# matssteinweg/Multi-Purpose-MPC

Measured on AMD Instinct MI355X. Metric: MPC QP solves/sec (batch, horizon N=30), higher is better.
Workload: dtype f64

## Files before the change

### multi-purpose-mpc_amd/csrc/mpmpc_reduced.hpp

```cpp
#pragma once
#include "mpmpc_core.hpp"

namespace mpmpc {

inline bool reduced_native(const mpmpc_config& c, const mpmpc_settings& st) {
  return st.native != 0 && reducible(c, st) && st.early_polish == 1 && st.max_iter > 1 && st.ipm_start_mu > 0.0 &&
         st.early_scaling >= 0 && st.scaling > 0;
}

template <class L, bool CR = true>
struct ReducedSolver : Solver<L, false, true, false, CR> {
  using S = Solver<L, false, true, false, CR>;
  using R = typename L::real;
  using Mk = typename L::mask;
  using I = typename L::ival;
  using S::N; using S::n_inst; using S::off_; using S::vx; using S::vu; using S::first; using S::down_chain; using S::is_mid;
  using S::is_end; using S::vxc; using S::sU; using S::val3; using S::bU; using S::live; using S::a; using S::b; using S::mI;
  using S::leq; using S::status; using S::iters; using S::ipm_iters; using S::polished; using S::pri_res; using S::dua_res;
  static constexpr bool kSplit = S::kSplit;
  static constexpr int LAY_RED = S::LAY_RED, LAY_REDSPLIT = S::LAY_REDSPLIT;
  static constexpr int LAY_IP = kSplit ? LAY_REDSPLIT : LAY_RED;
  static constexpr int EI = kSplit ? 2 : 3;
  using Box3 = typename S::template BoxT<LAY_RED>;
  using BoxI = typename S::template BoxT<LAY_IP>;
// ... 24 lines not shown
    n_inst = B;
    live = inst < B;
    vx = live & within_(k, 0, N);
    vu = live & within_(k, 0, N - 1);
    first = (k == 0);
    {
      const int C = L::split;
      off_ = lane_offset(L::group, C, N);
      I kl = k + off_;
      down_chain = (kl >= C);
      is_mid = (kl == C - 1);
      is_end = (kl == 2 * C - 1);
      I kc = seli(down_chain & (kl < 2 * C), kl * (-1) + (3 * C - 1), kl) - off_;
      vxc = live & within_(kc, 0, N);
      if constexpr (kSplit) {
        sU = (kl >= 32);
        Mk vU = live & within_(kl, 32 + off_, N + 31 + off_);
        val3[0] = selb(sU, vU, vx); val3[1] = selb(sU, vU, vx); val3[2] = vx & !sU;
      }
    }
    val[0] = vx; val[1] = vx; val[2] = vu;
  }
  MPMPC_HD void setup_problem(const R* fields, const SolverParams& st) {
    auto fld = [&](int f, double dflt) { return sel(vx, fields[f], R(dflt)); };
    const R zero(0.0), onec(1.0);
    const R lo_v = max_(fld(F_LO + 3, -INFTY), R(-INFTY)), hi_v = min_(fld(F_HI + 3, INFTY), R(INFTY));
    const R p_v = fld(F_P + 3, 1.0), q_v = fld(F_Q + 3, 0.0);
    R v = -q_v / p_v;
    v = sel((hi_v < R(INF_BOUND)) & (v > hi_v), hi_v, v);
    v = sel((lo_v > R(-INF_BOUND)) & (v < lo_v), lo_v, v);
    v = sel(vu, v, zero);
    L::cold_put(C_V, v);
    L::cold_put(C_LAMV, sel(vu, -fma_(p_v, v, q_v), zero));
    L::cold_put(C_A20, fld(F_A20, 0.0));
    L::cold_put(C_BV, fld(F_B20, 0.0) * v);
    L::cold_put(C_BEQ2, fld(F_BEQ + 2, 0.0));
    const R lo_e = max_(fld(F_LO + 0, -INFTY), R(-INFTY)), hi_e = min_(fld(F_HI + 0, INFTY), R(INFTY));
    const R lo_k = max_(fld(F_LO + 4, -INFTY), R(-INFTY)), hi_k = min_(fld(F_HI + 4, INFTY), R(INFTY));
    {
      R gap = max_(max_(sel(vx, lo_e - hi_e, zero), sel(vu, lo_k - hi_k, zero)), sel(vu, lo_v - hi_v, zero));
      gap = L::gmax(gap);
      empty = live & (gap > zero);
      solvable = live & !empty;
      L::cold_put(C_GAP, gap);
    }
    const R ds = fld(F_DS, 0.0), one = sel(vu, onec, zero);
    a[0] = one; a[1] = ds; a[2] = fld(F_A10, 0.0); a[3] = one;
    b[0] = ds;
    mI[0] = mI[1] = R(-1.0);
    P3[0] = fld(F_P + 0, 1.0); P3[1] = fld(F_P + 1, 1.0); P3[2] = fld(F_P + 4, 1.0);
    Q3[0] = fld(F_Q + 0, 0.0); Q3[1] = fld(F_Q + 1, 0.0); Q3[2] = fld(F_Q + 4, 0.0);
    R D3[3] = {onec, onec, onec}, G3[3] = {onec, onec, onec}, Eb[3] = {onec, onec, onec}, E2[2] = {onec, onec}, c3(1.0);
    const int passes = st.early_scaling > 0 && st.early_scaling < st.scaling ? st.early_scaling : st.scaling;
    const R inv_n_total(1.0 / double(3 * N + 2));
    for (int it = 0; it < passes; ++it) {
      R cn[3], rn[2], r_own[2];
      cn[0] = max_(max_(max_(abs_(P3[0]), abs_(mI[0])), max_(abs_(a[0]), abs_(a[2]))), abs_(G3[0]));
      cn[1] = max_(max_(max_(abs_(P3[1]), abs_(mI[1])), max_(abs_(a[1]), abs_(a[3]))), abs_(G3[1]));
      cn[2] = max_(max_(abs_(P3[2]), abs_(b[0])), abs_(G3[2]));
      r_own[0] = max_(abs_(a[0]), abs_(a[1]));
      r_own[1] = max_(max_(abs_(a[2]), abs_(a[3])), abs_(b[0]));
      R Dt[3], Et[2], Etb[3], Etd[2];
      MPMPC_UNROLL
      for (int i = 0; i < 2; ++i) {
        rn[i] = max_(abs_(mI[i]), L::up(r_own[i]));
        Et[i] = rsqrt_(S::limit(rn[i]));
        Etd[i] = L::down(Et[i]);
      }
      MPMPC_UNROLL
      for (int e = 0; e < 3; ++e) {
        Dt[e] = rsqrt_(S::limit(cn[e]));
        Etb[e] = rsqrt_(S::limit(abs_(G3[e])));
        P3[e] = (Dt[e] * P3[e]) * Dt[e];
        G3[e] = (Etb[e] * G3[e]) * Dt[e];
        Q3[e] = Dt[e] * Q3[e];
        D3[e] = D3[e] * Dt[e];
        Eb[e] = Eb[e] * Etb[e];
      }
      MPMPC_UNROLL
      for (int i = 0; i < 2; ++i) { mI[i] = (Et[i] * mI[i]) * Dt[i]; E2[i] = E2[i] * Et[i]; }
      a[0] = (Etd[0] * a[0]) * Dt[0]; a[1] = (Etd[0] * a[1]) * Dt[1];
      a[2] = (Etd[1] * a[2]) * Dt[0]; a[3] = (Etd[1] * a[3]) * Dt[1];
      b[0] = (Etd[1] * b[0]) * Dt[2];
      R s(0.0), mq(0.0);
      MPMPC_UNROLL
      for (int e = 0; e < 3; ++e) {
        s = s + sel(val[e], abs_(P3[e]), zero);
        mq = max_(mq, sel(val[e], abs_(Q3[e]), zero));
      }
      R ct = L::gsum(s) * inv_n_total;
      const R nq = S::limit(L::gmax(mq));
      ct = rcp_(S::limit(max_(ct, nq)));
      MPMPC_UNROLL
      for (int e = 0; e < 3; ++e) { P3[e] = P3[e] * ct; Q3[e] = Q3[e] * ct; }
      c3 = c3 * ct;
    }
    leq[0] = E2[0] * fld(F_BEQ + 0, 0.0);
    leq[1] = E2[1] * fld(F_BEQ + 1, 0.0);
    MPMPC_UNROLL
    for (int e = 0; e < 3; ++e) { L::cold_put(C_D + e, D3[e]); L::cold_put(C_G + e, G3[e]); }
    L::cold_put(C_E, E2[0]); L::cold_put(C_E + 1, E2[1]);
    L::cold_put(C_C, c3);
    {
      const R i0 = rcp_(D3[0]), i2 = rcp_(D3[2]);
      L::cold_put(K_LO0, lo_e * i0); L::cold_put(K_HI0, hi_e * i0); L::cold_put(K_LO2, lo_k * i2); L::cold_put(K_HI2, hi_k * i2);
    }
    MPMPC_UNROLL
    for (int e = 0; e < 3; ++e) {
      x3[e] = zero;
      L::cold_put(C_PI + e, zero);
    }
    L::fence();
  }

  MPMPC_HD void to_ip(const R v[3], R* o, double fill = 0.0) const {
    if constexpr (kSplit) {
      o[0] = sel(sU, L::from_lower(v[2]), v[0]);
      o[1] = sel(sU, R(fill), v[1]);
    } else {
      o[0] = v[0]; o[1] = v[1]; o[2] = v[2];
    }
  }
  MPMPC_HD void from_ip(const R* v, R o[3]) const {
    if constexpr (kSplit) {
      o[0] = v[0]; o[1] = v[1]; o[2] = L::from_upper(v[0]);
    } else {
      o[0] = v[0]; o[1] = v[1]; o[2] = v[2];
    }
  }
  MPMPC_HD void mask_to_ip(const Mk m[3], Mk* o) const {
    if constexpr (kSplit) {
      R v[3], w[2];
      MPMPC_UNROLL
      for (int e = 0; e < 3; ++e) v[e] = sel(m[e], R(1.0), R(0.0));
      to_ip(v, w);
      o[0] = w[0] > R(0.5); o[1] = w[1] > R(0.5);
    } else {
      o[0] = m[0]; o[1] = m[1]; o[2] = m[2];
    }
  }
  MPMPC_HD void mask_from_ip(const Mk* m, Mk o[3]) const {
    if constexpr (kSplit) {
      R w[2] = {sel(m[0], R(1.0), R(0.0)), sel(m[1], R(1.0), R(0.0))}, v[3];
      from_ip(w, v);
      MPMPC_UNROLL
      for (int e = 0; e < 3; ++e) o[e] = v[e] > R(0.5);
    } else {
      o[0] = m[0]; o[1] = m[1]; o[2] = m[2];
    }
  }

  template <bool SOFT = false>
  MPMPC_HD Mk ipm3(const Box3& bx, typename S::template IpmT<LAY_RED>& s, const SolverParams& st, double tol, const Mk& run, int band_slot = -1) {
    const R reg(st.ipm_reg), ireg(st.inv_ipm_reg), one(1.0), zero(0.0);
    constexpr int JB[2] = {0, 2};
    Mk active = run, conv = L::mfalse();
    R cnt(0.0);
    MPMPC_UNROLL
    for (int b = 0; b < 2; ++b) cnt = cnt + L::gcount(bx.Lm[JB[b]]) + L::gcount(bx.Um[JB[b]]);
    const R inb = rcp_(max_(cnt, one));
    I stall(0);
    R mu_min(1e300);
    auto lo_of = [&](int b) { return L::cold_get(b == 0 ? K_LO0 : K_LO2); };
    auto hi_of = [&](int b) { return L::cold_get(b == 0 ? K_HI0 : K_HI2); };
    auto iom_of = [&](int j) { const R gj = L::cold_get(C_G + j); return rcp_(gj * gj); };
    auto w_of = [&](int j) { return SOFT ? (s.zl[j] - s.zu[j]) * iom_of(j) : zero; };
    auto rl_of = [&](int b) { const int j = JB[b]; return SOFT ? s.x[j] + w_of(j) - lo_of(b) - s.sl[j] : s.x[j] - lo_of(b) - s.sl[j]; };
    auto ru_of = [&](int b) { const int j = JB[b]; return SOFT ? hi_of(b) - s.x[j] - w_of(j) - s.su[j] : hi_of(b) - s.x[j] - s.su[j]; };
    auto rpin_of = [&](int b) { const int j = JB[b]; return sel(bx.pin[j], s.x[j] - lo_of(b), zero); };
    auto rpin_raw = [&](int b) { const int j = JB[b]; return s.x[j] - lo_of(b); };
    for (int it = 0; it <= st.ipm_max_iter; ++it) {
      R mu;
      {
        L::fence();
        R At[3], rp[2], rd[3];
        this->template AeqT_mul_t<LAY_RED>(s.nu, At);
        this->template Aeq_mul_t<LAY_RED>(s.x, rp);
        R res(0.0), msum(0.0);
        MPMPC_UNROLL
        for (int i = 0; i < 2; ++i) {
          rp[i] = rp[i] - L::cold_get(K_LEQ + i);
          if constexpr (SOFT) rp[i] = fma_(R(-P1_EQ_SOFT), s.nu[i], rp[i]);
          res = max_(res, sel(vx, abs_(rp[i]), zero));
        }
        MPMPC_UNROLL
        for (int j = 0; j < 3; ++j) {
          if constexpr (SOFT) rd[j] = At[j] - s.zl[j] + s.zu[j] + s.pi[j];
          else rd[j] = fma_(L::cold_get(K_PP + j), s.x[j], L::cold_get(K_QQ + j)) + At[j] - s.zl[j] + s.zu[j] + s.pi[j];
        }
        res = max_(res, sel(val[1], abs_(rd[1]), zero));
        MPMPC_UNROLL
        for (int b = 0; b < 2; ++b) {
          const int j = JB[b];
          res = max_(res, sel(val[j], max_(max_(abs_(rd[j]), abs_(rpin_of(b))), max_(sel(bx.Lm[j], abs_(rl_of(b)), zero), sel(bx.Um[j], abs_(ru_of(b)), zero))), zero));
          msum = msum + s.sl[j] * s.zl[j] + s.su[j] * s.zu[j];
        }
        MPMPC_UNROLL
        for (int j = 0; j < 3; ++j) L::cold_put(K_RD + j, rd[j]);
        L::cold_put(K_RP, rp[0]); L::cold_put(K_RP + 1, rp[1]);
        res = L::gmax(res);
        mu = L::gsum(msum) * inb;
        Mk ok = (res < R(tol > 1e-11 ? tol : 1e-11)) & (mu < R(tol));
        if constexpr (SOFT) {
          S::p1_converged = selb(active, ok, S::p1_converged);
          R ny(0.0), na(0.0), sup(0.0);
          MPMPC_UNROLL
          for (int i = 0; i < 2; ++i) { ny = max_(ny, sel(vx, abs_(s.nu[i]), zero)); sup = sup + sel(vx, L::cold_get(K_LEQ + i) * s.nu[i], zero); }
          na = max_(na, sel(val[0], abs_(rd[0]), zero));
          na = max_(na, sel(val[1], abs_(rd[1]), zero));
          na = max_(na, sel(val[2], abs_(rd[2]), zero));
          MPMPC_UNROLL
          for (int b = 0; b < 2; ++b) {
            const int j = JB[b];
            const R lam = s.zu[j] - s.zl[j] + s.pi[j];
            ny = max_(ny, sel(val[j], abs_(lam), zero));
            sup = sup + sel(val[j] & (lam > zero) & (bx.Um[j] | bx.pin[j]), sel(bx.pin[j], lo_of(b), hi_of(b)) * lam, zero) +
                  sel(val[j] & (lam < zero) & (bx.Lm[j] | bx.pin[j]), lo_of(b) * lam, zero);
          }
          ny = L::gmax(ny); na = L::gmax(na); sup = L::gsum(sup);
          const R thr = R(st.phase1_eps) * ny;
          Mk ray = (ny > R(st.phase1_eps)) & (na < thr) & (sup < -thr);
          if (band_slot >= 0) {
            R wv(0.0);
            MPMPC_UNROLL
            for (int b = 0; b < 2; ++b) {
              const int j = JB[b];
              wv = max_(wv, sel(val[j], abs_(w_of(j)) * L::cold_get(C_D + j), zero));
            }
            ray = ray & (L::gmax(wv) > L::cold_get(band_slot));
          }
          ok = ok | ray;
        }
        conv = conv | (active & ok);
        active = active & !ok;
        if (it == st.ipm_max_iter || !L::wany(active)) break;
        if constexpr (!SOFT) {
          active = active & !(mu > R(st.ipm_diverged) * mu_min) & !((mu < R(tol * 1e-3)) & (res > R(1e-5)));
          mu_min = min_(mu_min, mu);
          if (!L::wany(active)) break;
        }
      }
      ipm_iters = seli(active, ipm_iters + I(1), ipm_iters);
      R isl[2], isu[2], rcl[2], rcu[2];
      [[maybe_unused]] R kap[2];
      {
        L::fence();
        R h[3];
        h[1] = SOFT ? rcp_(reg) : rcp_(L::cold_get(K_PP + 1) + reg);
        MPMPC_UNROLL
        for (int b = 0; b < 2; ++b) {
          const int j = JB[b];
          const R il = rcp_(s.sl[j]), iu = rcp_(s.su[j]);
          if constexpr (SOFT) {
            const R th = sel(bx.Lm[j], s.zl[j] * il, zero) + sel(bx.Um[j], s.zu[j] * iu, zero);
            const R kp = rcp_(fma_(th, iom_of(j), one));
            h[j] = rcp_(fma_(kp, th, reg) + sel(bx.pin[j], ireg, zero));
          } else {
            h[j] = rcp_(L::cold_get(K_PP + j) + reg + sel(bx.Lm[j], s.zl[j] * il, zero) + sel(bx.Um[j], s.zu[j] * iu, zero) +
                        sel(bx.pin[j], ireg, zero));
          }
        }
        this->template factor_t<LAY_RED>(h, SOFT ? reg + R(P1_EQ_SOFT) : reg);
        L::fence();
        MPMPC_UNROLL
        for (int b = 0; b < 2; ++b) {
          const int j = JB[b];
          isl[b] = sel(bx.Lm[j], rcp_(s.sl[j]), zero); isu[b] = sel(bx.Um[j], rcp_(s.su[j]), zero);
          rcl[b] = s.sl[j] * s.zl[j]; rcu[b] = s.su[j] * s.zu[j];
          if constexpr (SOFT) kap[b] = rcp_(fma_(s.zl[j] * isl[b] + s.zu[j] * isu[b], iom_of(j), one));
        }
      }
      R alpha_aff(1.0);
      for (int pass = 0; pass < 2; ++pass) {
        R dx[3], dnu[2];
        [[maybe_unused]] R cul[2];
        {
          L::fence();
          R rhs[3], nreq[2];
          rhs[1] = -L::cold_get(K_RD + 1);
          MPMPC_UNROLL
          for (int b = 0; b < 2; ++b) {
            const int j = JB[b];
            if constexpr (SOFT) {
              cul[b] = fma_(s.zu[j], ru_of(b), rcu[b]) * isu[b] - fma_(s.zl[j], rl_of(b), rcl[b]) * isl[b];
              rhs[j] = fma_(kap[b], cul[b], -L::cold_get(K_RD + j)) - sel(bx.pin[j], rpin_raw(b) * ireg, zero);
            } else {
              rhs[j] = -L::cold_get(K_RD + j) - fma_(s.zl[j], rl_of(b), rcl[b]) * isl[b] + fma_(s.zu[j], ru_of(b), rcu[b]) * isu[b] -
                       sel(bx.pin[j], rpin_raw(b) * ireg, zero);
            }
          }
          nreq[0] = -L::cold_get(K_RP); nreq[1] = -L::cold_get(K_RP + 1);
          this->template kkt_solve_t<LAY_RED>(rhs, nreq, dx, dnu);
          if (SOFT && pass == 1) {
            R Ad[2], Atd[3], r1[3], r2[2];
            this->template Aeq_mul_t<LAY_RED>(dx, Ad);
            this->template AeqT_mul_t<LAY_RED>(dnu, Atd);
            r1[1] = rhs[1] - Atd[1];
            MPMPC_UNROLL
            for (int b = 0; b < 2; ++b) {
              const int j = JB[b];
              r1[j] = rhs[j] - fma_(kap[b] * (s.zl[j] * isl[b] + s.zu[j] * isu[b]) + sel(bx.pin[j], ireg, zero), dx[j], Atd[j]);
            }
            r2[0] = fma_(R(P1_EQ_SOFT), dnu[0], nreq[0] - Ad[0]); r2[1] = fma_(R(P1_EQ_SOFT), dnu[1], nreq[1] - Ad[1]);
            L::fence();
            MPMPC_UNROLL
            for (int j = 0; j < 3; ++j) L::cold_put(K_RD + j, dx[j]);
// ... 403 lines not shown
```

### multi-purpose-mpc_amd/csrc/mpmpc_reduced_tail.hpp

```cpp
#pragma once
#include "mpmpc_reduced.hpp"

namespace mpmpc {

inline bool reduced_native_tail(const mpmpc_config& c, const mpmpc_settings& st) {
  return reduced_native(c, st) && st.phase1 != 0;
}

template <class L, bool CR = true>
struct ReducedTailSolver : ReducedSolver<L, CR> {
  using RS = ReducedSolver<L, CR>;
  using S = typename RS::S;
  using R = typename L::real;
  using Mk = typename L::mask;
  using I = typename L::ival;
  using S::N; using S::vx; using S::vu; using S::first; using S::live; using S::a; using S::b; using S::mI; using S::leq;
  using S::status; using S::iters; using S::ipm_iters; using S::polished; using S::pri_res; using S::dua_res;
  using S::sU; using S::val3; using S::bU;
  using RS::val; using RS::P3; using RS::Q3; using RS::x3; using RS::solvable; using RS::empty;
  using RS::C_D; using RS::C_E; using RS::C_C; using RS::K_LO0; using RS::K_HI0; using RS::K_LO2; using RS::K_HI2; using RS::C_V;
  using RS::C_LAMV; using RS::C_A20; using RS::C_BV; using RS::C_BEQ2; using RS::C_G; using RS::C_PI; using RS::C_XS; using RS::C_LAM;
  using RS::C_NUS; using RS::C_GAP;
  using Box3 = typename RS::Box3;
  using BoxI = typename RS::BoxI;
  using IpmI = typename RS::IpmI;
  static constexpr int EI = RS::EI;
  enum { T_RAW0 = 37, T_RAW1 = 38, T_RAW2 = 39, T_RAW3 = RS::C_PI, T_NAX = RS::C_PI + 1, T_RD0 = RS::C_PI + 2, T_MARK = RS::C_GAP,
         T_BAND = RS::C_NUS };
  static_assert(RS::K_RP + 2 <= 37, "the packed interior point's residual slots must end below T_RAW0");
  MPMPC_HD static constexpr int t_raw(int i) { return i == 0 ? T_RAW0 : (i == 1 ? T_RAW1 : (i == 2 ? T_RAW2 : T_RAW3)); }


  MPMPC_HD void setup_full(const R* fields, int B, const I& inst, const I& k, int N_, const SolverParams& st) {
    RS::context(B, inst, k, N_);
    auto fld = [&](int f, double dflt) { return sel(vx, fields[f], R(dflt)); };
    const R zero(0.0), onec(1.0);
    const R lo_v = max_(fld(F_LO + 3, -INFTY), R(-INFTY)), hi_v = min_(fld(F_HI + 3, INFTY), R(INFTY));
    const R p_v = fld(F_P + 3, 1.0), q_v = fld(F_Q + 3, 0.0);
    R v = -q_v / p_v;
    v = sel((hi_v < R(INF_BOUND)) & (v > hi_v), hi_v, v);
    v = sel((lo_v > R(-INF_BOUND)) & (v < lo_v), lo_v, v);
    v = sel(vu, v, zero);
    L::cold_put(C_V, v);
    L::cold_put(C_LAMV, sel(vu, -fma_(p_v, v, q_v), zero));
    L::cold_put(C_A20, fld(F_A20, 0.0));
    L::cold_put(C_BV, fld(F_B20, 0.0) * v);
    L::cold_put(C_BEQ2, fld(F_BEQ + 2, 0.0));
    const R lo_e = max_(fld(F_LO + 0, -INFTY), R(-INFTY)), hi_e = min_(fld(F_HI + 0, INFTY), R(INFTY));
    const R lo_k = max_(fld(F_LO + 4, -INFTY), R(-INFTY)), hi_k = min_(fld(F_HI + 4, INFTY), R(INFTY));
    {
      R gap = max_(max_(sel(vx, lo_e - hi_e, zero), sel(vu, lo_k - hi_k, zero)), sel(vu, lo_v - hi_v, zero));
      gap = L::gmax(gap);
      empty = live & (gap > zero);
      solvable = live & !empty;
      pri_res = gap;
      L::cold_put(T_MARK, zero);
    }
    {
      auto fin = [&](const R& bnd) { return sel(abs_(bnd) < R(INF_BOUND), abs_(bnd), zero); };
      R m = sel(vx, max_(fin(lo_e), fin(hi_e)), zero);
      m = max_(m, sel(vu, max_(max_(fin(lo_v), fin(hi_v)), max_(abs_(v), max_(fin(lo_k), fin(hi_k)))), zero));
      L::cold_put(T_NAX, L::gmax(m));
      R mb = sel(vx, max_(fin(lo_e), fin(hi_e)), zero);
      mb = max_(mb, sel(vu, max_(max_(fin(lo_v), fin(hi_v)), max_(fin(lo_k), fin(hi_k))), zero));
      L::cold_put(T_BAND, st.phase1_accept ? R(st.phase1_band) * fma_(R(st.eps_rel), L::gmax(mb), R(st.eps_abs)) : zero);
    }
    const R ds = fld(F_DS, 0.0), one = sel(vu, onec, zero);
    S::valid[0] = S::valid[1] = S::valid[2] = vx;
    S::valid[3] = S::valid[4] = vu;
    a[0] = one; a[1] = ds; a[2] = fld(F_A10, 0.0); a[3] = one; a[4] = fld(F_A20, 0.0); a[5] = one;
    b[0] = ds; b[1] = fld(F_B20, 0.0);
    MPMPC_UNROLL
    for (int i = 0; i < 3; ++i) { mI[i] = R(-1.0); S::Eeq[i] = onec; }
    MPMPC_UNROLL
    for (int j = 0; j < 5; ++j) {
      S::q[j] = fld(F_Q + j, 0.0);
      S::p[j] = fld(F_P + j, 1.0);
      S::g[j] = onec; S::D[j] = onec; S::Eb[j] = onec;
    }
    S::c = onec;
    const int passes = st.early_scaling > 0 && st.early_scaling < st.scaling ? st.early_scaling : st.scaling;
    S::ruiz(passes, live);
    constexpr int J5[3] = {0, 1, 4};
    MPMPC_UNROLL
    for (int e = 0; e < 3; ++e) {
      P3[e] = S::p[J5[e]]; Q3[e] = S::q[J5[e]];
      L::cold_put(C_D + e, S::D[J5[e]]);
      L::cold_put(C_G + e, S::g[J5[e]]);
      x3[e] = zero;
    }
    L::cold_put(T_RAW0, lo_e); L::cold_put(T_RAW1, hi_e); L::cold_put(T_RAW2, lo_k); L::cold_put(T_RAW3, hi_k);
    leq[0] = S::Eeq[0] * fld(F_BEQ + 0, 0.0);
    leq[1] = S::Eeq[1] * fld(F_BEQ + 1, 0.0);
    L::cold_put(C_E, S::Eeq[0]); L::cold_put(C_E + 1, S::Eeq[1]);
    L::cold_put(C_C, S::c);
    L::cold_put(K_LO0, (S::Eb[0] * lo_e) / S::g[0]); L::cold_put(K_HI0, (S::Eb[0] * hi_e) / S::g[0]);
    L::cold_put(K_LO2, (S::Eb[4] * lo_k) / S::g[4]); L::cold_put(K_HI2, (S::Eb[4] * hi_k) / S::g[4]);
    L::cold_put(T_RD0, L::gmax(sel(vu, abs_(fma_(S::p[3], v / S::D[3], S::q[3])), zero)));
    L::fence();
  }

  MPMPC_HD R violation(const R xs[3]) const {
    const R zero(0.0);
    R Ax[2], pv(0.0);
    this->template Aeq_mul_t<RS::LAY_RED>(xs, Ax);
    MPMPC_UNROLL
    for (int i = 0; i < 2; ++i) pv = max_(pv, sel(vx, abs_((Ax[i] - leq[i]) / L::cold_get(C_E + i)), zero));
    MPMPC_UNROLL
    for (int b2 = 0; b2 < 2; ++b2) {
      const int e = b2 == 0 ? 0 : 2;
      const R xu = L::cold_get(C_D + e) * xs[e];
      pv = max_(pv, sel(val[e], max_(max_(L::cold_get(t_raw(2 * b2)) - xu, xu - L::cold_get(t_raw(2 * b2 + 1))), zero), zero));
    }
    return L::gmax(pv);
  }

  MPMPC_HD void run(const R* fields, int B, const I& inst, const I& k, int N_, const SolverParams& st, const I& base_ipm) {
    MPMPC_TICK_BEGIN(0);
    setup_full(fields, B, inst, k, N_, st);
    MPMPC_TICK_END(0);
    const R zero(0.0), one(1.0);
    status = seli(empty, I(MPMPC_PRIMAL_INFEASIBLE), I(MPMPC_UNSOLVED));
    ipm_iters = base_ipm;
    polished = I(0);
    pri_res = sel(empty, pri_res, zero);
    dua_res = zero;
    this->act_bits = I(0);
    const Mk todo = solvable;
    if (L::wany(todo)) {
      Box3 b3;
      RS::make_box3(b3);
      R xs[3], lam[3], nus[2];
      {
        const R theta(st.phase1_theta);
        R sl[3], su[3], zl[3], zu[3];
        MPMPC_UNROLL
        for (int e = 0; e < 3; ++e) {
          const R ge = L::cold_get(C_G + e), ig = one / ge;
          sl[e] = sel(b3.Lm[e], max_(-(b3.lo[e] * ge), theta) * ig, one);
          su[e] = sel(b3.Um[e], max_(b3.hi[e] * ge, theta) * ig, one);
          zl[e] = sel(b3.Lm[e], theta * ge, zero);
          zu[e] = sel(b3.Um[e], theta * ge, zero);
        }
        BoxI bi;
        IpmI si;
        Mk vm[EI];
        if constexpr (RS::kSplit) {
          bU[0] = sel(sU, L::from_lower(b[0]), zero);
          bU[1] = zero;
          vm[0] = val3[0]; vm[1] = val3[2];
        } else {
          vm[0] = val[0]; vm[1] = val[1]; vm[2] = val[2];
        }
        RS::to_ip(b3.lo, bi.lo); RS::to_ip(b3.hi, bi.hi);
        RS::mask_to_ip(b3.Lm, bi.Lm); RS::mask_to_ip(b3.Um, bi.Um); RS::mask_to_ip(b3.pin, bi.pin);
        const R z3[3] = {zero, zero, zero};
        RS::to_ip(z3, si.x); RS::to_ip(sl, si.sl, 1.0); RS::to_ip(su, si.su, 1.0); RS::to_ip(zl, si.zl); RS::to_ip(zu, si.zu); RS::to_ip(z3, si.pi);
        si.nu[0] = si.nu[1] = zero;
        MPMPC_UNROLL
        for (int e = 0; e < EI; ++e) si.tL[e] = si.tU[e] = L::mfalse();
        S::p1_converged = L::mfalse();
        MPMPC_TICK_BEGIN(9);
        const double tol1 = st.ipm_tol * 1e-2 < 1e-11 ? st.ipm_tol * 1e-2 : 1e-11;
        if constexpr (RS::kSplit) {
          R om3[3], omI[EI];
          MPMPC_UNROLL
          for (int e = 0; e < 3; ++e) { const R ge = L::cold_get(C_G + e); om3[e] = ge * ge; }
          RS::to_ip(om3, omI, 1.0);
          R d3[3], dI[EI];
          MPMPC_UNROLL
          for (int e = 0; e < 3; ++e) d3[e] = L::cold_get(C_D + e) / om3[e];
          RS::to_ip(d3, dI, 1.0);
          S::p1_band = L::cold_get(T_BAND);
          this->template ipm<RS::LAY_IP, true>(bi, si, omI, dI, vm, st, tol1, todo);
        } else {
          MPMPC_UNROLL
          for (int e = 0; e < 3; ++e) { L::cold_put(RS::K_PP + e, P3[e]); L::cold_put(RS::K_QQ + e, Q3[e]); }
          L::cold_put(RS::K_LEQ, leq[0]); L::cold_put(RS::K_LEQ + 1, leq[1]);
          L::fence();
          RS::template ipm3<true>(bi, si, st, tol1, todo, st.phase1_accept ? (int)T_BAND : -1);
          L::fence();
          MPMPC_UNROLL
// ... 122 lines not shown
```

### multi-purpose-mpc_amd/csrc/mpmpc_solver_polish.hpp

```cpp
#ifndef MPMPC_SOLVER_BODY
#error "include mpmpc_core.hpp"
#endif
  template <int LAY>
  MPMPC_HD Mk active_set(const BoxT<LAY>& bx, const R* pp, const R* qq, const Mk* vm, Mk* aL, Mk* aU, R* xs, R* nus, R* lam,
                         const SolverParams& st, const Mk& run, double add_fraction) {
    constexpr int E = EN<LAY>, NQ = NR<LAY>;
    const R delta(st.as_delta), idelta(st.inv_as_delta), zero(0.0), one(1.0), tol(1e-9);
    Mk todo = run, okm = L::mfalse();
    for (int rnd = 0; rnd < st.as_rounds; ++rnd) {
      if (!L::wany(todo)) break;
      R bound[E];
      Mk act[E];
      MPMPC_UNROLL
      for (int j = 0; j < E; ++j) act[j] = aL[j] | aU[j] | bx.pin[j];
      {
        R h[E], Hd[E];
        MPMPC_UNROLL
        for (int j = 0; j < E; ++j) {
          Hd[j] = pp[j] + delta + sel(act[j], idelta, zero);
          h[j] = one / Hd[j];
        }
        dense_blocks<LAY>(Hd, h);
        MPMPC_TICK_COUNT(17);
        MPMPC_TICK_BEGIN(13);
        factor_t<LAY>(h, delta);
        MPMPC_TICK_END(13);
      }
      L::fence();
      MPMPC_UNROLL
      for (int j = 0; j < E; ++j) bound[j] = sel(aU[j], bx.hi[j], bx.lo[j]);
      R xn[E], nn[NQ], ln[E];
      MPMPC_UNROLL
      for (int j = 0; j < E; ++j) xn[j] = ln[j] = zero;
      MPMPC_UNROLL
      for (int i = 0; i < NQ; ++i) nn[i] = zero;
      [[maybe_unused]] Mk refine = todo;
      for (int rf = 0; rf <= st.as_refine; ++rf) {
        R At[E], Ax[NQ], rhs[E], r2[NQ], r3[E], dx[E], dnu[NQ];
        AeqT_mul_t<LAY>(nn, At);
        Aeq_mul_t<LAY>(xn, Ax);
        R rs(0.0);
        [[maybe_unused]] R Pod[E];
        if constexpr (FQ) {
          MPMPC_UNROLL
          for (int j = 0; j < E; ++j) Pod[j] = zero;
          Poff_add<LAY>(xn, Pod);
        }
        [[maybe_unused]] R rk_dot(0.0);
        if constexpr (LAY == LAY_RED4) rk_dot = rank_one_dot(xn);
        MPMPC_UNROLL
        for (int j = 0; j < E; ++j) {
          R r1 = -qq[j] - pp[j] * xn[j] - At[j] - ln[j];
          if constexpr (FQ) r1 = r1 - Pod[j];
          if constexpr (LAY == LAY_RED4) { if (j == 0 || j == 3) r1 = fma_(-rk_c[j == 0 ? 0 : 1], rk_dot, r1); }
          r3[j] = sel(act[j], bound[j] - xn[j], zero);
          rhs[j] = fma_(r3[j], idelta, r1);
          rs = max_(rs, sel(vm[j], max_(abs_(r1), abs_(r3[j])), zero));
        }
        MPMPC_UNROLL
        for (int i = 0; i < NQ; ++i) { r2[i] = leq[i] - Ax[i]; rs = max_(rs, sel(vx, abs_(r2[i]), zero)); }
        [[maybe_unused]] Mk need = todo;
        if constexpr (L::per_wave == 1) {
          if (rf >= 1 && !L::wany(todo & (L::gmax(rs) > R(1e-15)))) break;
        } else {
          if (rf >= 1) need = refine & (L::gmax(rs) > R(1e-15));
          if (!L::wany(need)) break;
        }
        MPMPC_TICK_COUNT(18);
        MPMPC_TICK_BEGIN(14);
        kkt_solve_t<LAY>(rhs, r2, dx, dnu);
        MPMPC_TICK_END(14);
        R big(0.0);
        MPMPC_UNROLL
        for (int j = 0; j < E; ++j) {
          ln[j] = updw(need, ln[j] + sel(act[j], (dx[j] - r3[j]) * idelta, zero), ln[j]);
          xn[j] = updw(need, xn[j] + dx[j], xn[j]);
          big = max_(big, sel(vm[j], abs_(dx[j]) - R(1e-14) * abs_(xn[j]), zero));
        }
        MPMPC_UNROLL
        for (int i = 0; i < NQ; ++i) nn[i] = updw(need, nn[i] + dnu[i], nn[i]);
        if constexpr (L::per_wave == 1) {
          if (rf >= 1 && !L::wany(todo & (L::gmax(big) > R(1e-15)))) break;
        } else {
          refine = rf < 1 ? need : need & (L::gmax(big) > R(1e-15));
          if (!L::wany(refine)) break;
        }
        if (L::per_wave == 1 && rf >= 1 && rf < st.as_refine) {
          const R far(1e-6);
          Mk clear = L::mfalse();
          MPMPC_UNROLL
          for (int j = 0; j < E; ++j)
            clear = clear | (bx.Lm[j] & !aL[j] & (xn[j] < bx.lo[j] - far)) | (bx.Um[j] & !aU[j] & (xn[j] > bx.hi[j] + far)) |
                    (aL[j] & (ln[j] > far)) | (aU[j] & (ln[j] < -far));
          if (!L::wany(todo & !L::gany(clear))) break;
        }
      }
      Mk anybad = L::mfalse();
      Mk vL[E], vU[E], bL[E], bU_[E];
      R worst(0.0);
      MPMPC_UNROLL
      for (int j = 0; j < E; ++j) {
        vL[j] = bx.Lm[j] & !aL[j] & (xn[j] < bx.lo[j] - tol);
        vU[j] = bx.Um[j] & !aU[j] & (xn[j] > bx.hi[j] + tol);
        bL[j] = aL[j] & (ln[j] > tol);
        bU_[j] = aU[j] & (ln[j] < -tol);
        anybad = anybad | vL[j] | vU[j] | bL[j] | bU_[j];
        worst = max_(worst, max_(sel(vL[j], bx.lo[j] - xn[j], zero), sel(vU[j], xn[j] - bx.hi[j], zero)));
      }
      anybad = L::gany(anybad);
      {
        const R thr = R(add_fraction) * L::gmax(worst);
        MPMPC_UNROLL
        for (int j = 0; j < E; ++j) {
          vL[j] = vL[j] & !(bx.lo[j] - xn[j] < thr);
          vU[j] = vU[j] & !(xn[j] - bx.hi[j] < thr);
        }
      }
      MPMPC_UNROLL
      for (int j = 0; j < E; ++j) {
        xs[j] = updw(todo, xn[j], xs[j]);
        lam[j] = updw(todo, ln[j], lam[j]);
        Mk nL = (aL[j] & !bL[j]) | vL[j];
        Mk nU = ((aU[j] & !bU_[j]) | vU[j]) & !nL;
        aL[j] = selb(todo & anybad, nL, aL[j]);
        aU[j] = selb(todo & anybad, nU, aU[j]);
      }
      MPMPC_UNROLL
      for (int i = 0; i < NQ; ++i) nus[i] = updw(todo, nn[i], nus[i]);
      okm = okm | (todo & !anybad);
      todo = todo & anybad;
    }
    return okm;
  }

  MPMPC_HD void reduced_complete(const Box& bx, R xs[5], R nus[3], R lam[5]) const {
    const R zero(0.0);
    R xv = -q[3] / p[3];
    xv = sel(bx.Um[3] & (xv > bx.hi[3]), bx.hi[3], xv);
    xv = sel((bx.Lm[3] | bx.pin[3]) & (xv < bx.lo[3]), bx.lo[3], xv);
    xv = sel(bx.pin[3], bx.lo[3], xv);
    xs[3] = sel(valid[3], xv, zero);
    lam[3] = sel(valid[3], -fma_(p[3], xs[3], q[3]), zero);
    nus[2] = zero;
    lam[2] = zero;
    const R imI = R(1.0) / mI[2], t0 = leq[2] * imI, drive = fma_(b[1], xs[3], a[4] * xs[0]);
    R t = t0;
    for (int it = 0; it < N; ++it) {
      const R inflow = L::up(fma_(a[5], t, drive));
      t = sel(first, t0, (leq[2] - inflow) * imI);
    }
    xs[2] = sel(vx, t, zero);
  }

  MPMPC_HD Mk certificate(const R xs[5], const R nus[3], const R lam[5], double tol, R& prim, R& stat) const {
    R Ax[3], At[5];
    Aeq_mul(xs, Ax);
    AeqT_mul(nus, At);
    R pv(0.0), sv(0.0), cv(0.0);
    R cinv = R(1.0) / c;
    R Pod[5] = {R(0.0), R(0.0), R(0.0), R(0.0), R(0.0)};
    if constexpr (FQ) Poff_add<0>(xs, Pod);
    MPMPC_UNROLL
    for (int i = 0; i < 3; ++i) pv = max_(pv, sel(vx, abs_((Ax[i] - leq[i]) / Eeq[i]), R(0.0)));
    MPMPC_UNROLL
    for (int j = 0; j < 5; ++j) {
      R xu = D[j] * xs[j];
      const R lo0 = lo_raw(j), hi0 = hi_raw(j);
      R viol = max_(max_(lo0 - xu, xu - hi0), R(0.0));
      pv = max_(pv, sel(valid[j], viol, R(0.0)));
      R rd = fma_(p[j], xs[j], q[j]) + At[j] + lam[j];
      if constexpr (FQ) rd = rd + Pod[j];
      sv = max_(sv, sel(valid[j], abs_(rd / D[j]) * cinv, R(0.0)));
      R yu = (lam[j] / D[j]) * cinv;
      Mk fu = hi0 < R(INF_BOUND), fl = lo0 > R(-INF_BOUND);
      R cu = sel(fu, max_(yu, R(0.0)) * abs_(hi0 - xu), sel(yu > R(0.0), R(1e300), R(0.0)));
      R cl = sel(fl, max_(-yu, R(0.0)) * abs_(xu - lo0), sel(yu < R(0.0), R(1e300), R(0.0)));
      cv = max_(cv, sel(valid[j], max_(cu, cl), R(0.0)));
    }
    Mk bad = L::mfalse();
    MPMPC_UNROLL
    for (int j = 0; j < 5; ++j) bad = bad | (valid[j] & !((abs_(xs[j]) < R(1e300)) & (abs_(lam[j]) < R(1e300))));
    MPMPC_UNROLL
    for (int i = 0; i < 3; ++i) bad = bad | (vx & !(abs_(nus[i]) < R(1e300)));
    bad = L::gany(bad);
    prim = L::gmax(pv);
    stat = L::gmax(sv);
    cv = L::gmax(cv);
    return (prim <= R(tol)) & (stat <= R(tol)) & (cv <= R(tol)) & !bad;
  }

  MPMPC_HD void stash() const {
    MPMPC_UNROLL
    for (int j = 0; j < 5; ++j) {
      L::cold_put(j, D[j]); L::cold_put(5 + j, Eb[j]); L::cold_put(10 + j, lb[j]); L::cold_put(15 + j, ub[j]);
      L::cold_put(20 + j, x[j]); L::cold_put(25 + j, yb[j]); L::cold_put(37 + j, g[j]);
    }
    MPMPC_UNROLL
    for (int i = 0; i < 3; ++i) { L::cold_put(30 + i, Eeq[i]); L::cold_put(33 + i, yeq[i]); }
    L::cold_put(36, c);
    L::fence();
  }
  MPMPC_HD void unstash() {
    L::fence();
    MPMPC_UNROLL
    for (int j = 0; j < 5; ++j) {
      D[j] = L::cold_get(j); Eb[j] = L::cold_get(5 + j); lb[j] = L::cold_get(10 + j); ub[j] = L::cold_get(15 + j);
      x[j] = L::cold_get(20 + j); yb[j] = L::cold_get(25 + j); g[j] = L::cold_get(37 + j);
    }
    MPMPC_UNROLL
    for (int i = 0; i < 3; ++i) { Eeq[i] = L::cold_get(30 + i); yeq[i] = L::cold_get(33 + i); }
    c = L::cold_get(36);
  }

  MPMPC_HD static I pack_active(const Mk aL[5], const Mk aU[5]) {
    I v(1 << 30);
    MPMPC_UNROLL
    for (int j = 0; j < 5; ++j) v = v + seli(aL[j], I(1 << j), I(0)) + seli(aU[j], I(32 << j), I(0));
    return v;
  }
  static constexpr int LAY_AS = RED ? LAY_RED : LAY_FULL;
  static constexpr int LAY_IP = RED ? (kSplit ? LAY_REDSPLIT : LAY_RED) : (kSplit ? LAY_SPLIT : LAY_FULL);

  template <int LAY>
  MPMPC_HD void problem_in_layout(const Box& bx, BoxT<LAY>& bi, R* pp, R* qq, Mk* vm) {
    constexpr int E = EN<LAY>;
    const R one(1.0), zero(0.0);
    if constexpr (SPL<LAY>) {
      MPMPC_UNROLL
      for (int i = 0; i < 2; ++i) bU[i] = sel(sU, L::from_lower(b[i]), zero);
      if constexpr (FQ) {
        podS[0] = sel(sU, L::from_lower(rod), pod[0]); podS[1] = sel(sU, zero, pod[1]); podS[2] = sel(sU, zero, pod[2]);
      }
    }
    to_lay<LAY>(bx.lo, bi.lo); to_lay<LAY>(bx.hi, bi.hi); to_lay<LAY>(p, pp); to_lay<LAY>(q, qq);
    mask_to_lay<LAY>(bx.Lm, bi.Lm); mask_to_lay<LAY>(bx.Um, bi.Um); mask_to_lay<LAY>(bx.pin, bi.pin);
    valid_lay<LAY>(vm);
    if constexpr (LAY == LAY_SPLIT) pp[2] = sel(sU, one, pp[2]);
    if constexpr (LAY == LAY_REDSPLIT) pp[1] = sel(sU, one, pp[1]);
    (void)E;
  }
  template <int LAY>
  MPMPC_HD void iterate_to_layout(const Ipm& s, IpmT<LAY>& si) const {
    const R one(1.0);
    to_lay<LAY>(s.x, si.x); to_lay<LAY>(s.sl, si.sl); to_lay<LAY>(s.su, si.su);
    to_lay<LAY>(s.zl, si.zl); to_lay<LAY>(s.zu, si.zu); to_lay<LAY>(s.pi, si.pi);
    if constexpr (LAY == LAY_SPLIT) { si.sl[2] = sel(sU, one, si.sl[2]); si.su[2] = sel(sU, one, si.su[2]); }
    if constexpr (LAY == LAY_REDSPLIT) { si.sl[1] = sel(sU, one, si.sl[1]); si.su[1] = sel(sU, one, si.su[1]); }
    MPMPC_UNROLL
    for (int i = 0; i < NR<LAY>; ++i) si.nu[i] = s.nu[i];
  }

  MPMPC_HD Mk active_set_full(const Box& bx, Mk aL5[5], Mk aU5[5], R xs[5], R nus[3], R lam[5], const SolverParams& st, double add_fraction,
                              const Mk& run) {
    constexpr int LAY = LAY_AS;
    constexpr int E = EN<LAY>, NQ = NR<LAY>;
    BoxT<LAY> ba;
    R pp[E], qq[E], xa[E], la[E], na[NQ];
    Mk vm[E], aL[E], aU[E];
    problem_in_layout<LAY>(bx, ba, pp, qq, vm);
    mask_to_lay<LAY>(aL5, aL); mask_to_lay<LAY>(aU5, aU);
    to_lay<LAY>(xs, xa); to_lay<LAY>(lam, la);
    MPMPC_UNROLL
    for (int i = 0; i < NQ; ++i) na[i] = nus[i];
    Mk okm = active_set<LAY>(ba, pp, qq, vm, aL, aU, xa, na, la, st, run, add_fraction);
    from_lay<LAY>(xa, xs); from_lay<LAY>(la, lam);
    MPMPC_UNROLL
    for (int i = 0; i < NQ; ++i) nus[i] = na[i];
    mask_from_lay<LAY>(aL, aL5); mask_from_lay<LAY>(aU, aU5);
    if constexpr (RED) {
      reduced_complete(bx, xs, nus, lam);
      aL5[2] = aU5[2] = L::mfalse();
      aL5[3] = bx.Lm[3] & (lam[3] < R(0.0)) & valid[3];
      aU5[3] = bx.Um[3] & (lam[3] > R(0.0)) & valid[3] & !aL5[3];
    }
    return okm;
  }

  MPMPC_HD void warm_polish(const SolverParams& st, const I& guess, const Mk& run) {
    Box bx;
    make_box(bx);
    Mk aL[5], aU[5];
    MPMPC_UNROLL
    for (int j = 0; j < 5; ++j) {
      aL[j] = bx.Lm[j] & bit_(guess, j);
// ... 139 lines not shown
```

Baseline: 70.44 million.

## Let each packed instance run its own active-set rounds independently within a wave

```diff
diff --git a/multi-purpose-mpc_amd/csrc/mpmpc_reduced.hpp b/multi-purpose-mpc_amd/csrc/mpmpc_reduced.hpp
--- a/multi-purpose-mpc_amd/csrc/mpmpc_reduced.hpp
+++ b/multi-purpose-mpc_amd/csrc/mpmpc_reduced.hpp
@@ -200,6 +200,7 @@
 
   template <bool SOFT = false>
   MPMPC_HD Mk ipm3(const Box3& bx, typename S::template IpmT<LAY_RED>& s, const SolverParams& st, double tol, const Mk& run, int band_slot = -1) {
+    static_assert(!(SOFT && kLean), "phase 1 needs the full cold storage");
     const R reg(st.ipm_reg), ireg(st.inv_ipm_reg), one(1.0), zero(0.0);
     constexpr int JB[2] = {0, 2};
     Mk active = run, conv = L::mfalse();
diff --git a/multi-purpose-mpc_amd/csrc/mpmpc_reduced_tail.hpp b/multi-purpose-mpc_amd/csrc/mpmpc_reduced_tail.hpp
--- a/multi-purpose-mpc_amd/csrc/mpmpc_reduced_tail.hpp
+++ b/multi-purpose-mpc_amd/csrc/mpmpc_reduced_tail.hpp
@@ -28,6 +28,7 @@
   enum { T_RAW0 = 37, T_RAW1 = 38, T_RAW2 = 39, T_RAW3 = RS::C_PI, T_NAX = RS::C_PI + 1, T_RD0 = RS::C_PI + 2, T_MARK = RS::C_GAP,
          T_BAND = RS::C_NUS };
   static_assert(RS::K_RP + 2 <= 37, "the packed interior point's residual slots must end below T_RAW0");
+  static_assert(!RS::kLean && T_RAW2 < L::cold_slots, "the tail solver needs the full cold storage: its own slots are the last three");
   MPMPC_HD static constexpr int t_raw(int i) { return i == 0 ? T_RAW0 : (i == 1 ? T_RAW1 : (i == 2 ? T_RAW2 : T_RAW3)); }
 
 
diff --git a/multi-purpose-mpc_amd/csrc/mpmpc_solver_polish.hpp b/multi-purpose-mpc_amd/csrc/mpmpc_solver_polish.hpp
--- a/multi-purpose-mpc_amd/csrc/mpmpc_solver_polish.hpp
+++ b/multi-purpose-mpc_amd/csrc/mpmpc_solver_polish.hpp
@@ -4,6 +4,7 @@
   template <int LAY>
   MPMPC_HD Mk active_set(const BoxT<LAY>& bx, const R* pp, const R* qq, const Mk* vm, Mk* aL, Mk* aU, R* xs, R* nus, R* lam,
                          const SolverParams& st, const Mk& run, double add_fraction) {
+    if constexpr (kOwnRounds) { return active_set_own<LAY>(bx, pp, qq, vm, aL, aU, xs, nus, lam, st, run, add_fraction); }
     constexpr int E = EN<LAY>, NQ = NR<LAY>;
     const R delta(st.as_delta), idelta(st.inv_as_delta), zero(0.0), one(1.0), tol(1e-9);
     Mk todo = run, okm = L::mfalse();
@@ -130,6 +131,143 @@
       okm = okm | (todo & !anybad);
       todo = todo & anybad;
     }
+    return okm;
+  }
+
+  static constexpr bool kOwnRounds = L::per_wave > 1 && !kS2;
+  template <int LAY>
+  MPMPC_HD Mk active_set_own(const BoxT<LAY>& bx, const R* pp, const R* qq, const Mk* vm, Mk* aL, Mk* aU, R* xs, R* nus, R* lam,
+                             const SolverParams& st, const Mk& run, double add_fraction) {
+    constexpr int E = EN<LAY>, NQ = NR<LAY>;
+    const R delta(st.as_delta), idelta(st.inv_as_delta), zero(0.0), one(1.0), tol(1e-9);
+    Mk todo = st.as_rounds > 0 ? run : L::mfalse(), okm = L::mfalse();
+    const Mk ran = todo;
+    Mk fresh = todo;
+    I rnd(0), rf(0);
+    R xn[E], nn[NQ], ln[E];
+    MPMPC_UNROLL
+    for (int j = 0; j < E; ++j) xn[j] = ln[j] = zero;
+    MPMPC_UNROLL
+    for (int i = 0; i < NQ; ++i) nn[i] = zero;
+    while (L::wany(todo)) {
+      Mk act[E];
+      MPMPC_UNROLL
+      for (int j = 0; j < E; ++j) act[j] = aL[j] | aU[j] | bx.pin[j];
+      if (L::wany(fresh)) {
+        {
+          R h[E], Hd[E];
+          MPMPC_UNROLL
+          for (int j = 0; j < E; ++j) {
+            Hd[j] = pp[j] + delta + sel(act[j], idelta, zero);
+            h[j] = one / Hd[j];
+          }
+          dense_blocks<LAY>(Hd, h);
+          MPMPC_TICK_COUNT(17);
+          MPMPC_TICK_BEGIN(13);
+          factor_t<LAY>(h, delta);
+          MPMPC_TICK_END(13);
+        }
+        L::fence();
+        MPMPC_UNROLL
+        for (int j = 0; j < E; ++j) { xn[j] = sel(fresh, zero, xn[j]); ln[j] = sel(fresh, zero, ln[j]); }
+        MPMPC_UNROLL
+        for (int i = 0; i < NQ; ++i) nn[i] = sel(fresh, zero, nn[i]);
+        rf = seli(fresh, I(0), rf);
+        fresh = L::mfalse();
+      }
+      R bound[E];
+      MPMPC_UNROLL
+      for (int j = 0; j < E; ++j) bound[j] = sel(aU[j], bx.hi[j], bx.lo[j]);
+      Mk ended;
+      {
+        R At[E], Ax[NQ], rhs[E], r2[NQ], r3[E], dx[E], dnu[NQ];
+        AeqT_mul_t<LAY>(nn, At);
+        Aeq_mul_t<LAY>(xn, Ax);
+        R rs(0.0);
+        [[maybe_unused]] R Pod[E];
+        if constexpr (FQ) {
+          MPMPC_UNROLL
+          for (int j = 0; j < E; ++j) Pod[j] = zero;
+          Poff_add<LAY>(xn, Pod);
+        }
+        [[maybe_unused]] R rk_dot(0.0);
+        if constexpr (LAY == LAY_RED4) rk_dot = rank_one_dot(xn);
+        MPMPC_UNROLL
+        for (int j = 0; j < E; ++j) {
+          R r1 = -qq[j] - pp[j] * xn[j] - At[j] - ln[j];
+          if constexpr (FQ) r1 = r1 - Pod[j];
+          if constexpr (LAY == LAY_RED4) { if (j == 0 || j == 3) r1 = fma_(-rk_c[j == 0 ? 0 : 1], rk_dot, r1); }
+          r3[j] = sel(act[j], bound[j] - xn[j], zero);
+          rhs[j] = fma_(r3[j], idelta, r1);
+          rs = max_(rs, sel(vm[j], max_(abs_(r1), abs_(r3[j])), zero));
+        }
+        MPMPC_UNROLL
+        for (int i = 0; i < NQ; ++i) { r2[i] = leq[i] - Ax[i]; rs = max_(rs, sel(vx, abs_(r2[i]), zero)); }
+        const Mk need = todo & !(rf > st.as_refine) & ((rf < 1) | (L::gmax(rs) > R(1e-15)));
+        ended = todo & !need;
+        if (L::wany(need)) {
+          MPMPC_TICK_COUNT(18);
+          MPMPC_TICK_BEGIN(14);
+          kkt_solve_t<LAY>(rhs, r2, dx, dnu);
+          MPMPC_TICK_END(14);
+          R big(0.0);
+          MPMPC_UNROLL
+          for (int j = 0; j < E; ++j) {
+            ln[j] = updw(need, ln[j] + sel(act[j], (dx[j] - r3[j]) * idelta, zero), ln[j]);
+            xn[j] = updw(need, xn[j] + dx[j], xn[j]);
+            big = max_(big, sel(vm[j], abs_(dx[j]) - R(1e-14) * abs_(xn[j]), zero));
+          }
+          MPMPC_UNROLL
+          for (int i = 0; i < NQ; ++i) nn[i] = updw(need, nn[i] + dnu[i], nn[i]);
+          const Mk conv = (rf >= 1) & !(L::gmax(big) > R(1e-15));
+          const R far(1e-6);
+          Mk clear = L::mfalse();
+          MPMPC_UNROLL
+          for (int j = 0; j < E; ++j)
+            clear = clear | (bx.Lm[j] & !aL[j] & (xn[j] < bx.lo[j] - far)) | (bx.Um[j] & !aU[j] & (xn[j] > bx.hi[j] + far)) |
+                    (aL[j] & (ln[j] > far)) | (aU[j] & (ln[j] < -far));
+          ended = ended | (need & (conv | (rf >= st.as_refine) | ((rf >= 1) & (rf < st.as_refine) & L::gany(clear))));
+          rf = seli(need, rf + 1, rf);
+        }
+      }
+      if (!L::wany(ended)) continue;
+      Mk anybad = L::mfalse();
+      Mk vL[E], vU[E], bL[E], bU_[E];
+      R worst(0.0);
+      MPMPC_UNROLL
+      for (int j = 0; j < E; ++j) {
+        vL[j] = bx.Lm[j] & !aL[j] & (xn[j] < bx.lo[j] - tol);
+        vU[j] = bx.Um[j] & !aU[j] & (xn[j] > bx.hi[j] + tol);
+        bL[j] = aL[j] & (ln[j] > tol);
+        bU_[j] = aU[j] & (ln[j] < -tol);
+        anybad = anybad | vL[j] | vU[j] | bL[j] | bU_[j];
+        worst = max_(worst, max_(sel(vL[j], bx.lo[j] - xn[j], zero), sel(vU[j], xn[j] - bx.hi[j], zero)));
+      }
+      anybad = L::gany(anybad);
+      {
+        const R thr = R(add_fraction) * L::gmax(worst);
+        MPMPC_UNROLL
+        for (int j = 0; j < E; ++j) {
+          vL[j] = vL[j] & !(bx.lo[j] - xn[j] < thr);
+          vU[j] = vU[j] & !(xn[j] - bx.hi[j] < thr);
+        }
+      }
+      MPMPC_UNROLL
+      for (int j = 0; j < E; ++j) {
+        Mk nL = (aL[j] & !bL[j]) | vL[j];
+        Mk nU = ((aU[j] & !bU_[j]) | vU[j]) & !nL;
+        aL[j] = selb(ended & anybad, nL, aL[j]);
+        aU[j] = selb(ended & anybad, nU, aU[j]);
+      }
+      okm = okm | (ended & !anybad);
+      rnd = seli(ended, rnd + 1, rnd);
+      todo = todo & !(ended & (!anybad | !(rnd < st.as_rounds)));
+      fresh = ended & todo;
+    }
+    MPMPC_UNROLL
+    for (int j = 0; j < E; ++j) { xs[j] = sel(ran, xn[j], xs[j]); lam[j] = sel(ran, ln[j], lam[j]); }
+    MPMPC_UNROLL
+    for (int i = 0; i < NQ; ++i) nus[i] = sel(ran, nn[i], nus[i]);
     return okm;
   }
 
diff --git a/profiles/packed_rounds/rounds_census.py b/profiles/packed_rounds/rounds_census.py
--- /dev/null
+++ b/profiles/packed_rounds/rounds_census.py
@@ -0,0 +1,84 @@
+import argparse
+import ctypes as C
+import os
+import sys
+
+import numpy as np
+
+ROOT = os.path.dirname(os.path.dirname(os.path.dirname(os.path.abspath(__file__))))
+for d in ("multi-purpose-mpc_amd", "tests", ""):
+    sys.path.insert(0, os.path.join(ROOT, d))
+import mpmpc
+import mpmpc_testlib as tl
+import scenarios
+
+
+def scenario(config, B, seed=None):
+    spec = scenarios.CONFIGS[config]
+    keep = spec["seed"]
+    try:
+        if seed is not None:
+            spec["seed"] = seed
+        return scenarios.make(config, scenarios.sim_track(), B)
+    finally:
+        spec["seed"] = keep
+
+
+def counts(emu, cfg, st, qp, G):
+    out = (C.c_longlong * 32)()
+    emu.lib.emu_event_counts(out, 1)
+    sol, _ = emu.solve_rn(cfg, st, qp, G=G)
+    emu.lib.emu_event_counts(out, 1)
+    return sol, out[17], out[18]
+
+
+def census(emu, config, B, seed=None):
+    tr = scenarios.sim_track()
+    sc = scenario(config, B, seed)
+    cfg = tl.stock_config(sc.N, weights=sc.weights)
+    st = mpmpc.default_settings()
+    qp = emu.assemble(cfg, tr, (sc.wp_id, sc.x0, sc.cc_prev, sc.lb, sc.ub), obstacles=sc.obstacles)
+    rounds = np.zeros(B, int)
+    for i in range(B):
+        _, f, _ = counts(emu, cfg, st, np.ascontiguousarray(qp[:, i:i + 1]), 64)
+        rounds[i] = f
+    waves = []
+    for w in range(0, B, 2):
+        _, f, s = counts(emu, cfg, st, np.ascontiguousarray(qp[:, w:w + 2]), 32)
+        waves.append((w // 2, int(rounds[w]), int(rounds[min(w + 1, B - 1)]), f, s))
+    return np.array(waves), rounds
+
+
+if __name__ == "__main__":
+    ap = argparse.ArgumentParser()
+    ap.add_argument("--config", type=int, default=2)
+    ap.add_argument("--batch", type=int, default=0)
+    ap.add_argument("--seed", type=int, default=None)
+    ap.add_argument("--emul", default=None, help="another build's libmpmpc_emul.so")
+    ap.add_argument("--waves", action="store_true")
+    ap.add_argument("--dump-qp", default=None, metavar="FILE", help="write the batch for rounds_sanitize.cpp and stop")
+    a = ap.parse_args()
+    emu = tl.Emul()
+    if a.emul:
+        emu.lib = C.CDLL(os.path.abspath(a.emul))
+    B = a.batch or scenarios.CONFIGS[a.config]["B"]
+    if a.dump_qp:
+        sc = scenario(a.config, B, a.seed)
+        cfg, st = tl.stock_config(sc.N, weights=sc.weights), mpmpc.default_settings()
+        qp = emu.assemble(cfg, scenarios.sim_track(), (sc.wp_id, sc.x0, sc.cc_prev, sc.lb, sc.ub), obstacles=sc.obstacles)
+        with open(a.dump_qp, "wb") as f:
+            f.write(np.array([sc.N, B, C.sizeof(cfg), C.sizeof(st)], np.int32).tobytes() + bytes(cfg) + bytes(st) +
+                    np.ascontiguousarray(qp).tobytes())
+        sys.exit(0)
+    w, rounds = census(emu, a.config, B, a.seed)
+    multi = (w[:, 1] > 1).astype(int) + (w[:, 2] > 1).astype(int)
+    one = multi == 1
+    print("config %d seed %s B %d: %d waves, factorisations %d, solves %d; instances by rounds %s; waves with exactly one "
+          "multi-round instance %d (factorisations %d, solves %d), with two %d (factorisations %d, solves %d), others: "
+          "factorisations %d, solves %d" %
+          (a.config, a.seed, B, len(w), w[:, 3].sum(), w[:, 4].sum(), dict(zip(*np.unique(rounds, return_counts=True))),
+           one.sum(), w[one, 3].sum(), w[one, 4].sum(), (multi == 2).sum(), w[multi == 2, 3].sum(), w[multi == 2, 4].sum(),
+           w[multi == 0, 3].sum(), w[multi == 0, 4].sum()))
+    if a.waves:
+        for r in w[multi > 0]:
+            print("  wave %4d: rounds %d | %d, factorisations %d, solves %d" % tuple(r))
diff --git a/profiles/packed_rounds/rounds_sanitize.cpp b/profiles/packed_rounds/rounds_sanitize.cpp
--- /dev/null
+++ b/profiles/packed_rounds/rounds_sanitize.cpp
@@ -0,0 +1,33 @@
+#include "emul.cpp"
+#include <cstdio>
+int main(int argc, char** argv) {
+  if (argc < 2) { std::printf("usage: rounds_sanitize FILE\n"); return 2; }
+  std::FILE* f = std::fopen(argv[1], "rb");
+  if (!f) { std::printf("cannot open %s\n", argv[1]); return 2; }
+  int head[4];
+  mpmpc_config cfg;
+  mpmpc_settings st;
+  if (std::fread(head, sizeof(int), 4, f) != 4 || head[2] != (int)sizeof cfg || head[3] != (int)sizeof st ||
+      std::fread(&cfg, sizeof cfg, 1, f) != 1 || std::fread(&st, sizeof st, 1, f) != 1) { std::printf("bad header\n"); return 2; }
+  const int N = head[0], B = head[1], ld = stage_ld(N), n = 5 * N + 3, m = 8 * N + 6;
+  std::vector<double> qp((size_t)MPMPC_NUM_FIELDS * B * ld);
+  if (cfg.N != N || std::fread(qp.data(), sizeof(double), qp.size(), f) != qp.size()) { std::printf("bad problem\n"); return 2; }
+  std::fclose(f);
+  std::vector<double> z[2], u0[2], rs[2], y[2];
+  std::vector<int> status[2], iters[2];
+  long long cnt[2][32];
+  for (int r = 0; r < 2; ++r) {
+    z[r].assign((size_t)B * n, 0.0); u0[r].assign((size_t)B * 2, 0.0); rs[r].assign((size_t)B * 2, 0.0); y[r].assign((size_t)B * m, 0.0);
+    status[r].assign(B, 0); iters[r].assign((size_t)B * 2, 0);
+    int n_tail = 0;
+    emu_event_counts(cnt[r], 1);
+    if (emu_solve_rn(&cfg, &st, r == 0 ? 32 : 64, qp.data(), B, z[r].data(), u0[r].data(), status[r].data(), iters[r].data(), rs[r].data(),
+                     y[r].data(), &n_tail)) { std::printf("solve failed\n"); return 1; }
+    emu_event_counts(cnt[r], 1);
+    std::printf("%d lanes per instance: %lld factorisations, %lld active-set solves, %d left to the tail\n", r == 0 ? 32 : 64, cnt[r][17],
+                cnt[r][18], n_tail);
+  }
+  const bool same = z[0] == z[1] && u0[0] == u0[1] && status[0] == status[1] && iters[0] == iters[1] && y[0] == y[1];
+  std::printf("%d instances, N = %d: the two packings %s\n", B, N, same ? "agree bit for bit" : "DIFFER");
+  return same ? 0 : 1;
+}
```

After: 68.95 million. 0.979x the previous value.
